# zhangyu2ustc/GCN_fmri_decoding

Hardware: AMD Instinct MI355X
Metric: fMRI-windows/sec (fwd+bwd) 6-layer ChebNet K=5 N≈10k; HBM GB/s vs roofline (higher is better)
Workload: dtype f32; 1 GPU; BASELINE configs[1]: ChebNet K=5 x6 conv (F=32, p=1, b2relu), FC 512-256-22, synthetic N=10000 kNN-8 graph -> M=10466, block_dura=15, batch 64 per GPU; global_batch=64, parallelism=dp1, step=fwd+loss+bwd+allreduce+Adam, batch gathered on device

## Files before the change

### gcn_fmri_decoding_amd/_lib.py

```python
import ctypes as C
import os

_HERE = os.path.dirname(os.path.abspath(__file__))
LIB_PATH = os.environ.get('CHEBGCN_LIB') or os.path.join(_HERE, 'libchebgcn.so')

BIAS_NONE, BIAS_FILTER, BIAS_VERTEX = 0, 1, 2
POOL_MAX, POOL_AVG = 0, 1
KNN_EUCLIDEAN, KNN_COSINE, KNN_CORRELATION, KNN_DOT = 0, 1, 2, 3
KNN_KMAX = 32
PARCEL_MEAN, PARCEL_SUM = 0, 1


class ChebgcnError(RuntimeError):
    pass


_p = C.c_void_p
_i = C.c_int
_i64 = C.c_int64
_f = C.c_float

SIGNATURES = {
    'chebgcn_version': (_i, []),
    'chebgcn_last_error': (C.c_char_p, []),
    'chebgcn_last_dispatch': (C.c_char_p, []),
    'chebgcn_plane_stride': (_i, [_i]),
    'chebgcn_graph_create': (_i, [_i, _i64, _p, _p, _p, C.POINTER(_p)]),
    'chebgcn_graph_create_planes': (_i, [_i, _i64, _p, _p, _p, _i, C.POINTER(_p)]),
    'chebgcn_graph_destroy': (None, [_p]),
    'chebgcn_graph_query': (_i, [_p, _i, C.POINTER(_i64)]),
    'chebgcn_recurrence_fwd': (_i, [_p, _p, _p, _i, _i, _i, _p]),
    'chebgcn_recurrence_bwd': (_i, [_p, _p, _p, _i, _i, _i, _p]),
    'chebgcn_recurrence_fwd_t': (_i, [_p, _p, _p, _i, _i, _i, _p]),
    'chebgcn_reindex_weights': (_i, [_p, _p, _i, _i, _i, _p]),
    'chebgcn_reindex_weights_batch': (_i, [_i, _p, _p, _p, _p, _p, _p]),
    'chebgcn_contract_fwd': (_i, [_p, _p, _p, _i, _p, _p, _i, _i, _i, _i, _i, _i, _i, _i, _p]),
    'chebgcn_contract_fwd_windows_supported': (_i, [_i, _i, _i, _i, _i, _i]),
    'chebgcn_contract_fwd_windows': (_i, [_p, _i64, _p, _p, _p, _i, _p, _p, _i, _i, _i, _i, _i, _i, _i, _i, _p]),
    'chebgcn_contract_fwd_bf16_workspace': (C.c_size_t, [_i, _i, _i]),
    'chebgcn_contract_fwd_bf16': (_i, [_p, _p, _p, _i, _p, _p, _i, _i, _i, _i, _i, _i, _i, _i, _i, _p, C.c_size_t, _p]),
    'chebgcn_contract_bwd_x_bf16_workspace': (C.c_size_t, [_i, _i, _i]),
    'chebgcn_contract_bwd_x_bf16': (_i, [_p, _p, _p, _i, _i, _i, _i, _i, _i, _p, C.c_size_t, _p]),
    'chebgcn_contract_bwd_w_bf16_workspace': (C.c_size_t, [_i, _i, _i, _i, _i]),
    'chebgcn_contract_bwd_w_bf16': (_i, [_p, _p, _p, _p, C.c_size_t, _i, _i, _i, _i, _i, _i, _p]),
    'chebgcn_adam_partials': (_i, [_i64]),
    'chebgcn_adam_step_sq': (_i, [_p, _p, _p, _p, _i64, _f, _p, _f, _f, _f, _f, _f, _p, _p]),
    'chebgcn_adam_step_sq_all': (_i, [_p, _p, _p, _p, _i64, _i64, _f, _p, _f, _f, _f, _f, _f, _p, _p]),
    'chebgcn_nadam_step_sq_all': (_i, [_p, _p, _p, _p, _i64, _i64, _f, _p, _f, _f, _f, _f, _f, _p, _p]),
    'chebgcn_loss_bookkeeping': (_i, [_p, _p, _i, _f, _p, _f, _f, _p, _p, _p, _p]),
    'chebgcn_set_scalars': (_i, [_p, C.c_float, C.c_float, _p]),
    'chebgcn_softmax_xent': (_i, [_p, _p, _i, _p, _p, _i, _i, _p]),
    'chebgcn_relu_grad_bf16': (_i, [_p, _p, _p, _p, _i, _i, _i, _i, _p, C.c_size_t, _p]),
    'chebgcn_bf16_dy16_supported': (_i, [_i, _i, _i, _i, _i]),
    'chebgcn_contract_bwd_w_bf16_dy16': (_i, [_p, _p, _p, _p, C.c_size_t, _i, _i, _i, _i, _i, _p]),
    'chebgcn_contract_bwd_x_bf16_dy16': (_i, [_p, _p, _p, _i, _i, _i, _i, _i, _p, C.c_size_t, _p]),
    'chebgcn_brelu_pool_fwd': (_i, [_p, _p, _i, _p, _p, _i, _i, _i, _i, _i, _i, _p]),
    'chebgcn_brelu_pool_bwd_workspace': (C.c_size_t, [_i, _i, _i, _i, _i]),
    'chebgcn_brelu_pool_bwd': (_i, [_p, _p, _p, _p, _p, _i, _i, _i, _i, _i, _i, _i, _p, C.c_size_t, _p]),
    'chebgcn_pool_gather_fwd': (_i, [_p, _p, _p, _p, _i, _i, _i, _i, _i, _i, _p]),
    'chebgcn_pool_scatter_bwd_workspace': (C.c_size_t, [_i, _i, _i, _i, _i]),
    'chebgcn_pool_scatter_bwd': (_i, [_p, _p, _p, _p, _p, _i, _i, _i, _i, _i, _i, _i, _p, C.c_size_t, _p]),
    'chebgcn_contract_bwd_w_workspace': (C.c_size_t, [_i, _i, _i, _i, _i]),
    'chebgcn_contract_bwd_w': (_i, [_p, _p, _p, _p, C.c_size_t, _i, _i, _i, _i, _i, _p]),
    'chebgcn_contract_bwd_x': (_i, [_p, _p, _p, _i, _i, _i, _i, _i, _p]),
    'chebgcn_contract_bwd_x_relu': (_i, [_p, _p, _p, _p, _i, _i, _i, _i, _i, _p]),
    'chebgcn_contract_bwd_w_relu': (_i, [_p, _p, _p, _p, _p, C.c_size_t, _i, _i, _i, _i, _i, _p]),
    'chebgcn_contract_bwd_w_relu_bias_merged': (_i, [_i, _i, _i, _i, _i]),
    'chebgcn_contract_bwd_w_relu_bias': (_i, [_p, _p, _p, _p, _p, _p, C.c_size_t, _i, _i, _i, _i, _i, _p]),
    'chebgcn_contract_fwd_mean_supported': (_i, [_i, _i, _i, _i, _i]),
    'chebgcn_contract_fwd_gated_supported': (_i, [_i, _i, _i, _i, _i]),
    'chebgcn_contract_fwd_gated': (_i, [_p, _p, _p, _p, _i, _i, _i, _i, _i, _p]),
    'chebgcn_contract_fwd_mean': (_i, [_p, _p, _p, _i, _p, _p, _i, _i, _i, _i, _i, _p]),
    'chebgcn_contract_bwd_w_relu_mean': (_i, [_p, _p, _p, _p, _p, C.c_size_t, _i, _i, _i, _i, _i, _p]),
    'chebgcn_contract_bwd_x_relu_mean': (_i, [_p, _p, _p, _p, _i, _i, _i, _i, _i, _p]),
    'chebgcn_bias_grad_relu_mean': (_i, [_p, _p, _p, _i, _i, _i, _i, _p, C.c_size_t, _p]),
    'chebgcn_relu_grad_mean': (_i, [_p, _p, _p, _p, _i, _i, _i, _i, _p, C.c_size_t, _p]),
    'chebgcn_fused_layer_supported': (_i, [_p, _i, _i, _i, _i]),
    'chebgcn_fused_layer_workspace': (C.c_size_t, [_p, _i, _i, _i, _i]),
    'chebgcn_fused_layer_fwd': (_i, [_p, _p, _p, _p, _i, _p, _p, _p, _p, C.c_size_t, _i, _i, _i, _i, _i, _p]),
    'chebgcn_fused_layer_bwd_x': (_i, [_p, _p, _p, _p, _p, _i, _i, _i, _i, _p]),
    'chebgcn_perm_data': (_i, [_p, _p, _p, _p, _i, _i, _i, _i, _p]),
    'chebgcn_to_plane': (_i, [_p, _p, _i, _i, _i, _p]),
    'chebgcn_from_plane': (_i, [_p, _p, _i, _i, _i, _p]),
    'chebgcn_feature_mean_fwd': (_i, [_p, _p, _i, _i, _i, _p]),
    'chebgcn_feature_mean_bwd': (_i, [_p, _p, _i, _i, _i, _p]),
    'chebgcn_fc_fwd_supported': (_i, [_i, _i, _i]),
    'chebgcn_fc_fwd_workspace': (C.c_size_t, [_i, _i, _i]),
    'chebgcn_fc_fwd': (_i, [_p, _i64, _p, _p, _p, _p, C.c_size_t, _i, _i, _i, _i, _p]),
    'chebgcn_fc_bwd': (_i, [_p, _i64, _p, _p, _p, _p, _p, _p, _i64, _i, _i, _i, _p]),
    'chebgcn_planes_to_rows': (_i, [_p, _p, _p, _i, _i, _i, _i64, _p]),
    'chebgcn_rows_to_planes': (_i, [_p, _p, _p, _i, _i, _i, _i64, _p]),
    'chebgcn_adam_step': (_i, [_p, _p, _p, _p, _i64, _f, _f, _f, _f, _f, _f, _p]),
    'chebgcn_adam_step_dev': (_i, [_p, _p, _p, _p, _i64, _p, _f, _f, _f, _f, _f, _p]),
    'chebgcn_metis_one_level_f32': (_i, [_i64, _p, _p, _p, _p, _p, _i64, _p]),
    'chebgcn_metis_one_level_f32p': (_i, [_i64, _p, _p, _p, _p, _p, _i64, _p]),
    'chebgcn_metis_one_level_f64': (_i, [_i64, _p, _p, _p, _p, _p, _i64, _p]),
    'chebgcn_compute_perm_level': (_i, [_p, _i64, _p, _i64, _p]),
    'chebgcn_bank_order': (_i, [_i, _p, _p, _i, _p, _p]),
    'chebgcn_spectral_transform': (_i, [_p, _p, _p, _i, _i, _i, _p]),
    'chebgcn_spectral_mix_fwd': (_i, [_p, _p, _p, _i, _i, _i, _i, _p]),
    'chebgcn_spectral_mix_bwd_x': (_i, [_p, _p, _p, _i, _i, _i, _i, _p]),
    'chebgcn_spectral_mix_bwd_w': (_i, [_p, _p, _p, _i, _i, _i, _i, _p]),
    'chebgcn_spectral_spline_expand': (_i, [_p, _p, _p, _i, _i, _i, _p]),
    'chebgcn_spectral_spline_expand_bwd': (_i, [_p, _p, _p, _i, _i, _i, _p]),
    'chebgcn_saliency_supported': (_i, [_i]),
    'chebgcn_saliency_seed': (_i, [_p, _p, _i, _i, _i, _p, _p, _i, _i, _p]),
    'chebgcn_saliency_path': (_i, [_p, _p, _p, _p, _p, _i, _i, _i, _i, _i, _i, _p]),
    'chebgcn_saliency_reduce': (_i, [_p, _p, _p, _p, _p, _i, _i, _i, _i, _i, _i, _p, _p, _i, _p, _p]),
    'chebgcn_occlusion_supported': (_i, [_i]),
    'chebgcn_occlusion_rows': (_i, [_p, _p, _p, _p, _p, _i64, _i, _i, _i, _i, _i, _i, _p]),
    'chebgcn_occlusion_score': (_i, [_p, _i64, _i, _i, _i, _i, _p, _i, _p, _p, _p]),
    'chebgcn_occlusion_class_sums': (_i, [_p, _p, _i, _i, _i, _p, _p]),
    'chebgcn_gradcam_weights': (_i, [_p, _i, _i, _i, _p, _p]),
    'chebgcn_gradcam_map': (_i, [_p, _p, _p, _p, _i, _i, _i, _i, _i, _p, _i64, _p]),
    'chebgcn_gather_windows': (_i, [_p, _i64, _p, _p, _p, _p, _p, _i, _i, _i, _p]),
    'chebgcn_gather_windows_mix': (_i, [_p, _i64, _p, _p, _i, _p, _p, _p, _p, _i, _i, _i, _p]),
    'chebgcn_window_stats_workspace': (C.c_size_t, [_i64, _i, _i]),
    'chebgcn_window_stats': (_i, [_p, _i64, _p, _i64, _p, _p, _p, _p, _i, _i, _p, C.c_size_t, _p]),
    'chebgcn_gather_windows_indexed': (_i, [_p, _i64, _p, _i64, _i, _i, _p, _p, _i64, _i, _p, _p, _p, _p, _i, _i, _i, _p]),
    'chebgcn_window_stats_indexed_workspace': (C.c_size_t, [_i64, _i, _i]),
    'chebgcn_window_stats_indexed': (_i, [_p, _i64, _p, _i64, _i, _i, _p, _p, _p, _p, _i, _i, _p, C.c_size_t, _p]),
    'chebgcn_knn_workspace': (C.c_size_t, [_i, _i, _i]),
    'chebgcn_knn': (_i, [_p, _i, _i, _i, _i, _p, _p, _p, C.c_size_t, _p]),
    'chebgcn_series_normalise': (_i, [_p, _i64, _p, _i, _i, _f, _p, _p]),
    'chebgcn_parcellate_query': (_i, [_i]),
    'chebgcn_parcellate': (_i, [_p, _i64, _p, _p, _i64, _p, _p, _i64, _i64, _i, _i, _i, _p]),
    'chebgcn_parcel_expand': (_i, [_p, _p, _p, _i64, _i, _i, _f, _p]),
}

_lib = None


def lib():
    global _lib
    if _lib is None:
        if not os.path.exists(LIB_PATH):
            raise ChebgcnError(
                'libchebgcn.so not found at %s: build it with '
                '`python -c "import __graft_entry__ as g; g.build()"` or '
                '`make -C gcn_fmri_decoding_amd/csrc` (needs hipcc, --offload-arch=gfx950). '
                'There is no CPU fallback.' % LIB_PATH)
        import torch
        handle = C.CDLL(LIB_PATH)
        for name, (res, args) in SIGNATURES.items():
            fn = getattr(handle, name)
            fn.restype = res
            fn.argtypes = args
        _lib = handle
    return _lib


dispatch_log = None


def check(rc, what):
    if rc != 0:
        msg = lib().chebgcn_last_error()
        raise ChebgcnError('%s failed (%d): %s' % (what, rc, msg.decode() if msg else '?'))
    if dispatch_log is not None:
        dispatch_log.append((what, lib().chebgcn_last_dispatch().decode()))


def last_dispatch():
    return lib().chebgcn_last_dispatch().decode()


def plane_stride(M):
    return (int(M) + 31) & ~31
```

### gcn_fmri_decoding_amd/csrc/head.hip

```cpp
#include <hip/hip_runtime.h>
#include "../../include/chebgcn.h"
#include "status.h"
#include "contract_common.h"

namespace chebgcn {

constexpr int FC_WAVES = 8;
constexpr int FC_CHUNK = 32;
constexpr int FC_U = 2;

__global__ void __launch_bounds__(FC_WAVES * 64)
fc_fwd_kernel(const float* __restrict__ x, long long ldx, const float* __restrict__ W, const float* __restrict__ bias,
              float* __restrict__ y, float* __restrict__ part_out, int B, int I, int O, int relu, int cps) {
    __shared__ float part[FC_WAVES][32][33];
    const int lane = threadIdx.x & 63, wave = threadIdx.x >> 6;
    const int c = lane & 31, h = lane >> 5;
    const int bx = blockIdx.x, by = blockIdx.y, bz = blockIdx.z;
    const int o0 = bx * 32, b0 = by * 32;
    const int brow = min(b0 + c, B - 1), ocol = min(o0 + c, O - 1);
    const float* xr = x + (size_t)brow * ldx;
    const float* wc = W + ocol;
    const int nchunks = (I + FC_CHUNK - 1) / FC_CHUNK;
    const int q_lo = bz * cps, q_hi = min(q_lo + cps, nchunks);
    f32x16 acc;
// ... 97 lines not shown
                const int b = 8 * (wave + FC_WAVES * (q0 + u)) + 4 * h + j;
                const bool ok = b < B;
                const float gm = (ok && yv[u][j] > 0.f) ? gv[u][j] : 0.f;
                bsum += gm;
                acc = __builtin_amdgcn_mfma_f32_32x32x2f32(ok ? av[u][j] : 0.f, gm, acc, 0, 0, 0);
            }
    }
#pragma unroll
    for (int j = 0; j < 16; ++j) part[wave][acc_row(j, h)][c] = acc[j];
    bpart[wave][h][c] = bsum;
    __syncthreads();
    for (int e = threadIdx.x; e < 32 * 32; e += FC_WAVES * 64) {
        const int r = e >> 5, cc = e & 31;
        float s = part[0][r][cc];
#pragma unroll
        for (int w = 1; w < FC_WAVES; ++w) s += part[w][r][cc];
        if (i0 + r < I && o0 + cc < O) dW[(size_t)(i0 + r) * O + o0 + cc] = s;
    }
    if (db && blockIdx.y == 0 && threadIdx.x < 32 && o0 + threadIdx.x < O) {
        float s = 0.f;
#pragma unroll
        for (int w = 0; w < FC_WAVES; ++w) s += bpart[w][0][threadIdx.x] + bpart[w][1][threadIdx.x];
        db[o0 + threadIdx.x] = s;
    }
}

template <bool VEC>
__global__ void __launch_bounds__(FC_WAVES * 64)
fc_bwd_x_kernel(const float* __restrict__ g, const float* __restrict__ y, const float* __restrict__ W,
                float* __restrict__ dx, long long lddx, int B, int I, int O) {
    __shared__ float part[FC_WAVES][32][33];
    const int lane = threadIdx.x & 63, wave = threadIdx.x >> 6;
    const int c = lane & 31, h = lane >> 5;
    const int i0 = blockIdx.x * 32, b0 = blockIdx.y * 32;
    const int brow = min(b0 + c, B - 1), irow = min(i0 + c, I - 1);
    const float* gr = g + (size_t)brow * O;
    const float* yr = y ? y + (size_t)brow * O : nullptr;
    const float* wr = W + (size_t)irow * O;
    const int nchunks = (O + 7) >> 3;
    f32x16 acc;
#pragma unroll
    for (int j = 0; j < 16; ++j) acc[j] = 0.f;
    constexpr int U = 4;
    for (int q0 = 0; wave + FC_WAVES * q0 < nchunks; q0 += U) {
        f32x4 gv[U], yv[U], wv[U];
#pragma unroll
        for (int u = 0; u < U; ++u) {
            const int k = 8 * (wave + FC_WAVES * (q0 + u)) + 4 * h;
            if (VEC) {
                const int kc = k < O ? k : 0;
                gv[u] = *reinterpret_cast<const f32x4*>(gr + kc);
                wv[u] = *reinterpret_cast<const f32x4*>(wr + kc);
                if (yr) yv[u] = *reinterpret_cast<const f32x4*>(yr + kc);
            } else {
#pragma unroll
                for (int j = 0; j < 4; ++j) {
                    const int kc = k + j < O ? k + j : 0;
                    gv[u][j] = gr[kc];
                    wv[u][j] = wr[kc];
                    if (yr) yv[u][j] = yr[kc];
                }
            }
        }
#pragma unroll
        for (int u = 0; u < U; ++u) {
            const int k = 8 * (wave + FC_WAVES * (q0 + u)) + 4 * h;
#pragma unroll
            for (int j = 0; j < 4; ++j) {
                const bool ok = k + j < O;
                const float gm = (ok && (!yr || yv[u][j] > 0.f)) ? gv[u][j] : 0.f;
                acc = __builtin_amdgcn_mfma_f32_32x32x2f32(gm, ok ? wv[u][j] : 0.f, acc, 0, 0, 0);
            }
        }
    }
#pragma unroll
    for (int j = 0; j < 16; ++j) part[wave][acc_row(j, h)][c] = acc[j];
    __syncthreads();
    for (int e = threadIdx.x; e < 32 * 32; e += FC_WAVES * 64) {
        const int r = e >> 5, cc = e & 31;
        float s = part[0][r][cc];
#pragma unroll
        for (int w = 1; w < FC_WAVES; ++w) s += part[w][r][cc];
        if (b0 + r < B && i0 + cc < I) dx[(size_t)(b0 + r) * lddx + i0 + cc] = s;
    }
}

constexpr int FLAT_V = 64;
template <bool TO_ROWS>
__global__ void __launch_bounds__(256)
planes_rows_kernel(const float* __restrict__ src, float* __restrict__ dst, const int* __restrict__ order, int M, int Mp, int F,
                   long long ldr) {
    __shared__ float tile[32][FLAT_V + 1];
    const int b = blockIdx.y, v0 = blockIdx.x * FLAT_V;
    const int nv = max(0, min(FLAT_V, M - v0));
    const int nall = min(FLAT_V, Mp - v0);
    for (int f0 = 0; f0 < F; f0 += 32) {
        const int nf = min(32, F - f0);
        if (TO_ROWS) {
            for (int e = threadIdx.x; e < 32 * FLAT_V; e += 256) {
                const int f = e / FLAT_V, vl = e % FLAT_V;
                if (f < nf && vl < nv) tile[f][vl] = src[((size_t)b * F + f0 + f) * Mp + v0 + vl];
            }
            __syncthreads();
            for (int e = threadIdx.x; e < nf * nv; e += 256) {
                const int vl = e / nf, f = e % nf;
                const int m = order ? order[v0 + vl] : v0 + vl;
                dst[(size_t)b * ldr + (size_t)m * F + f0 + f] = tile[f][vl];
            }
        } else {
            for (int e = threadIdx.x; e < nf * nv; e += 256) {
                const int vl = e / nf, f = e % nf;
                const int m = order ? order[v0 + vl] : v0 + vl;
                tile[f][vl] = src[(size_t)b * ldr + (size_t)m * F + f0 + f];
            }
            __syncthreads();
            for (int e = threadIdx.x; e < 32 * FLAT_V; e += 256) {
                const int f = e / FLAT_V, vl = e % FLAT_V;
                if (f < nf && vl < nall) dst[((size_t)b * F + f0 + f) * Mp + v0 + vl] = vl < nv ? tile[f][vl] : 0.f;
            }
        }
        __syncthreads();
    }
}

}

namespace chebgcn {
constexpr int XENT_REG = 32;
template <typename LabelT>
__global__ void __launch_bounds__(256)
softmax_xent_kernel(const float* __restrict__ z, const LabelT* __restrict__ y, float* __restrict__ loss,
                    float* __restrict__ dz, int B, int C) {
    __shared__ float part[256];
    float acc = 0.f;
    const float invB = 1.f / (float)B;
    for (int b = threadIdx.x; b < B; b += 256) {
        const float* row = z + (size_t)b * C;
        long long t = (long long)y[b];
        const bool bad = t < 0 || t >= C;
        t = t < 0 ? 0 : t >= C ? C - 1 : t;
        float* drow = dz + (size_t)b * C;
        if (bad) {
            acc += __builtin_nanf("");
            for (int c = 0; c < C; ++c) drow[c] = __builtin_nanf("");
            continue;
        }
        if (C <= XENT_REG) {
            float v[XENT_REG];
#pragma unroll
            for (int c = 0; c < XENT_REG; ++c) v[c] = c < C ? row[c] : -__builtin_inff();
            float m = v[0];
#pragma unroll
            for (int c = 1; c < XENT_REG; ++c) m = fmaxf(m, v[c]);
            float s = 0.f, so = 0.f, et = 0.f;
#pragma unroll
            for (int c = 0; c < XENT_REG; ++c) {
                v[c] = c < C ? expf(v[c] - m) : 0.f;
                s += v[c];
                so += c == t ? 0.f : v[c];
                et = c == t ? v[c] : et;
            }
            acc += et > 1e-30f ? log1pf(so / et) : logf(s) - logf(fmaxf(et, 1e-45f));
            const float inv = invB / s;
#pragma unroll
            for (int c = 0; c < XENT_REG; ++c)
                if (c < C) drow[c] = c == t ? -so * inv : v[c] * inv;
// ... 6 lines not shown
            const float e = expf(row[c] - m);
            s += e;
            so += c == t ? 0.f : e;
        }
        const float et = expf(row[t] - m);
        acc += et > 1e-30f ? log1pf(so / et) : logf(s) - (row[t] - m);
        const float inv = invB / s;
        for (int c = 0; c < C; ++c) drow[c] = c == t ? -so * inv : expf(row[c] - m) * inv;
    }
    part[threadIdx.x] = acc;
    __syncthreads();
    for (int d = 128; d > 0; d >>= 1) {
        if ((int)threadIdx.x < d) part[threadIdx.x] += part[threadIdx.x + d];
        __syncthreads();
    }
    if (threadIdx.x == 0) *loss = part[0] * invB;
}
}

using namespace chebgcn;

static int fc_splits(int B, int I, int O) {
    const int tiles = ((O + 31) / 32) * ((B + 31) / 32);
    int s = 512 / tiles;
    const int by_len = (I + 511) / 512;
    if (s > by_len) s = by_len;
    return s < 1 ? 1 : s;
}

extern "C" int chebgcn_fc_fwd_supported(int B, int I, int O) {
    return B > 0 && I > 0 && O > 0 && I <= (1 << 20) && (long long)B * O <= (1 << 20);
}

extern "C" size_t chebgcn_fc_fwd_workspace(int B, int I, int O) {
    if (!chebgcn_fc_fwd_supported(B, I, O)) return 0;
    const int S = fc_splits(B, I, O);
    return S > 1 ? (size_t)S * B * O * sizeof(float) : 0;
}

extern "C" int chebgcn_fc_fwd(const float* x, int64_t ldx, const float* W, const float* bias, float* y, void* workspace,
                              size_t workspace_bytes, int B, int I, int O, int relu, chebgcn_stream stream_) {
    hipStream_t stream = (hipStream_t)stream_;
    CG_REQUIRE(x && W && y && B > 0 && I > 0 && O > 0 && ldx >= I, "fc_fwd: bad argument");
    if (!chebgcn_fc_fwd_supported(B, I, O) || (ldx & 3) || ((uintptr_t)x & 15))
        return CHEBGCN_EUNSUPPORTED;
    const int S = fc_splits(B, I, O);
    const int nchunks = (I + FC_CHUNK - 1) / FC_CHUNK, cps = (nchunks + S - 1) / S;
    CG_REQUIRE(S == 1 || (workspace && workspace_bytes >= chebgcn_fc_fwd_workspace(B, I, O)), "fc_fwd: workspace too small");
    dim3 grid((O + 31) / 32, (B + 31) / 32, S);
    note_dispatch(S > 1 ? "fc_fwd_kernel<split>" : "fc_fwd_kernel");
    if (S > 1) note_dispatch_more("fc_fwd_reduce_kernel");
    hipLaunchKernelGGL(fc_fwd_kernel, grid, dim3(FC_WAVES * 64), 0, stream, x, (long long)ldx, W, bias, y,
                       S > 1 ? (float*)workspace : nullptr, B, I, O, relu, cps);
    if (S > 1)
        hipLaunchKernelGGL(fc_fwd_reduce_kernel, dim3((B * O + 255) / 256), dim3(256), 0, stream, (const float*)workspace, bias,
                           y, B * O, O, S, relu);
    CG_HIP(hipGetLastError());
    return CHEBGCN_OK;
}

extern "C" int chebgcn_fc_bwd(const float* x, int64_t ldx, const float* W, const float* g, const float* y, float* dW,
                              float* db, float* dx, int64_t lddx, int B, int I, int O, chebgcn_stream stream_) {
    hipStream_t stream = (hipStream_t)stream_;
    CG_REQUIRE(x && W && g && B > 0 && I > 0 && O > 0 && ldx >= I && (!dx || lddx >= I), "fc_bwd: bad argument");
    if (!chebgcn_fc_fwd_supported(B, I, O)) return CHEBGCN_EUNSUPPORTED;
    note_dispatch(dW ? "fc_bwd_w_kernel" : "");
    if (dW) {
        dim3 grid((O + 31) / 32, (I + 31) / 32);
        hipLaunchKernelGGL(fc_bwd_w_kernel, grid, dim3(FC_WAVES * 64), 0, stream, x, (long long)ldx, g, y, dW, db, B, I, O);
    }
    if (dx) {
        dim3 grid((I + 31) / 32, (B + 31) / 32);
        const bool vec = (O & 3) == 0 && ((uintptr_t)g & 15) == 0 && ((uintptr_t)W & 15) == 0 && (!y || ((uintptr_t)y & 15) == 0);
        note_dispatch_more(vec ? "fc_bwd_x_kernel<true>" : "fc_bwd_x_kernel<false>");
        if (vec)
            hipLaunchKernelGGL(fc_bwd_x_kernel<true>, grid, dim3(FC_WAVES * 64), 0, stream, g, y, W, dx, (long long)lddx, B, I, O);
        else
            hipLaunchKernelGGL(fc_bwd_x_kernel<false>, grid, dim3(FC_WAVES * 64), 0, stream, g, y, W, dx, (long long)lddx, B, I, O);
    }
    CG_HIP(hipGetLastError());
    return CHEBGCN_OK;
}

static int planes_rows(bool to_rows, const float* src, float* dst, const int32_t* order, int B, int M, int F, int64_t ldr,
                       hipStream_t stream) {
    CG_REQUIRE(src && dst && B > 0 && B <= 65535 && M > 0 && F > 0 && ldr >= (int64_t)M * F,
               to_rows ? "planes_to_rows: bad argument" : "rows_to_planes: bad argument");
    const int Mp = plane_stride(M);
    dim3 grid(((to_rows ? M : Mp) + FLAT_V - 1) / FLAT_V, B);
    note_dispatch(to_rows ? "planes_rows_kernel<to_rows>" : "planes_rows_kernel<to_planes>");
    if (to_rows)
        hipLaunchKernelGGL(planes_rows_kernel<true>, grid, dim3(256), 0, stream, src, dst, order, M, Mp, F, (long long)ldr);
    else
        hipLaunchKernelGGL(planes_rows_kernel<false>, grid, dim3(256), 0, stream, src, dst, order, M, Mp, F, (long long)ldr);
    CG_HIP(hipGetLastError());
    return CHEBGCN_OK;
}

extern "C" int chebgcn_planes_to_rows(const float* planes, float* rows, const int32_t* order, int B, int M, int F, int64_t ldr,
                                      chebgcn_stream stream) {
    return planes_rows(true, planes, rows, order, B, M, F, ldr, (hipStream_t)stream);
}

extern "C" int chebgcn_rows_to_planes(const float* rows, float* planes, const int32_t* order, int B, int M, int F, int64_t ldr,
                                      chebgcn_stream stream) {
    return planes_rows(false, rows, planes, order, B, M, F, ldr, (hipStream_t)stream);
}

extern "C" int chebgcn_softmax_xent(const float* logits, const void* labels, int labels_int64, float* loss, float* dlogits,
                                    int B, int C, chebgcn_stream stream_) {
    hipStream_t stream = (hipStream_t)stream_;
    CG_REQUIRE(logits && labels && loss && dlogits, "softmax_xent: NULL argument");
    CG_REQUIRE(B > 0 && C > 0, "softmax_xent: bad shape");
    note_dispatch(labels_int64 ? "softmax_xent_kernel<int64>" : "softmax_xent_kernel<int32>");
    if (labels_int64)
        hipLaunchKernelGGL(softmax_xent_kernel<long long>, dim3(1), dim3(256), 0, stream, logits, (const long long*)labels, loss,
                           dlogits, B, C);
    else
        hipLaunchKernelGGL(softmax_xent_kernel<int32_t>, dim3(1), dim3(256), 0, stream, logits, (const int32_t*)labels, loss,
                           dlogits, B, C);
    CG_HIP(hipGetLastError());
    return CHEBGCN_OK;
}
```

### gcn_fmri_decoding_amd/ops.py

```python
import ctypes as C
import os
import weakref

import numpy as np
import scipy.sparse as sp
import torch

from . import _lib
from . import graph as _graph
from ._lib import BIAS_FILTER, BIAS_NONE, BIAS_VERTEX, POOL_AVG, POOL_MAX, plane_stride


def _stream():
    return C.c_void_p(torch.cuda.current_stream().cuda_stream)


def _p(t):
    return C.c_void_p(t.data_ptr()) if t is not None else None


class KernelTimers:

    def __init__(self, every=1, by_dispatch=False):
        self.records = {}
# ... 1001 lines not shown
    return out


def spectral_mix_bwd_w(dyh, xh, M):
    B, Fout, Mp = dyh.shape
    Fin = xh.shape[1]
    dW = torch.empty((M, Fout, Fin), dtype=torch.float32, device=dyh.device)
    _launch('spectral_mix_bwd_w', 4.0 * (B * (Fin + Fout) * Mp + dW.numel()), 2.0 * B * M * Fin * Fout,
            lambda: _lib.check(_lib.lib().chebgcn_spectral_mix_bwd_w(_p(dyh), _p(xh), _p(dW), B, M, Fin, Fout, _stream()),
                               'spectral_mix_bwd_w'))
    return dW


def spline_expand(Bs, Wk, transpose=False):
    M, K = Bs.shape
    C = Wk.shape[1]
    if transpose:
        out = torch.empty((K, C), dtype=torch.float32, device=Wk.device)
        fn, what = _lib.lib().chebgcn_spectral_spline_expand_bwd, 'spectral_spline_expand_bwd'
    else:
        out = torch.empty((M, C), dtype=torch.float32, device=Wk.device)
        fn, what = _lib.lib().chebgcn_spectral_spline_expand, 'spectral_spline_expand'
    _launch(what, 4.0 * (M * K + (M + K) * C), 2.0 * M * K * C,
            lambda: _lib.check(fn(_p(Bs), _p(Wk), _p(out), M, K, C, _stream()), what))
    return out


class SpectralConv(torch.autograd.Function):

    @staticmethod
    def forward(ctx, x, W, basis, Bs, M, Fout):
        _require_cuda(x, W, basis, Bs)
        x = x if x.is_contiguous() else x.contiguous()
        B, Fin, Mp = x.shape
        if basis.shape != (Mp, Mp):
            raise ValueError('spectral conv: basis %s for planes of %d vertices' % (tuple(basis.shape), M))
        Wd = W.detach().contiguous()
        Wf = (spline_expand(Bs, Wd) if Bs is not None else Wd).view(M, Fout, Fin)
        xh = spectral_transform(x, basis, M, False)
        y = spectral_transform(spectral_mix(xh, Wf, M), basis, M, True)
        ctx.save_for_backward(xh if ctx.needs_input_grad[1] else None, Wf, basis, Bs)
        ctx.M = M
        return y

    @staticmethod
    def backward(ctx, gy):
        xh, Wf, basis, Bs = ctx.saved_tensors
        M = ctx.M
        gy = gy if gy.is_contiguous() else gy.contiguous()
        dyh = spectral_transform(gy, basis, M, False)
        dx = dW = None
        if ctx.needs_input_grad[1]:
            dW = spectral_mix_bwd_w(dyh, xh, M)
            if Bs is not None:
                dW = spline_expand(Bs, dW.view(M, -1), transpose=True)
        if ctx.needs_input_grad[0]:
            dx = spectral_transform(spectral_mix(dyh, Wf, M, transpose=True), basis, M, True)
        return dx, dW, None, None, None, None


class FeatureMean(torch.autograd.Function):

    @staticmethod
    def forward(ctx, x, M):
        _require_cuda(x)
        x = x if x.is_contiguous() else x.contiguous()
        B, F, Mp = x.shape
        y = torch.empty((B, M), dtype=torch.float32, device=x.device)
        _lib.check(_lib.lib().chebgcn_feature_mean_fwd(_p(x), _p(y), B, M, F, _stream()), 'feature_mean_fwd')
        ctx.cfg = (B, M, F, Mp)
        return y

    @staticmethod
    def backward(ctx, gy):
        B, M, F, Mp = ctx.cfg
        gy = gy.contiguous()
        dx = torch.empty((B, F, Mp), dtype=torch.float32, device=gy.device)
        _lib.check(_lib.lib().chebgcn_feature_mean_bwd(_p(gy), _p(dx), B, M, F, _stream()), 'feature_mean_bwd')
        return dx, None


FC_BWD_MAX_INNER = int(os.environ.get('CHEBGCN_FC_BWD_MAX_INNER', 4096))
FC_FWD_MAX_INNER = int(os.environ.get('CHEBGCN_FC_FWD_MAX_INNER', 1 << 20))


def fc_forward(x, W, b, relu):
    if not (x.is_cuda and x.dtype == torch.float32 and W.dtype == torch.float32 and x.dim() == 2 and W.is_contiguous()
            and x.stride(1) == 1 and x.stride(0) % 4 == 0 and x.data_ptr() % 16 == 0):
        return None
    B, I = x.shape
    O = W.shape[1]
    L = _lib.lib()
    if I > FC_FWD_MAX_INNER or not L.chebgcn_fc_fwd_supported(B, I, O):
        return None
    y = torch.empty((B, O), dtype=torch.float32, device=x.device)
    nws = L.chebgcn_fc_fwd_workspace(B, I, O)
    ws = _workspace(nws, x.device, 'fc_fwd') if nws else None
    _lib.check(L.chebgcn_fc_fwd(_p(x), x.stride(0), _p(W), _p(b), _p(y), _p(ws), nws, B, I, O, 1 if relu else 0, _stream()),
               'fc_fwd')
    return y


def fc_backward(x, W, g, y, dW, db, need_dx):
    B, I = x.shape
    O = W.shape[1]
    L = _lib.lib()
    if not (x.is_cuda and x.dtype == torch.float32 and x.stride(1) == 1 and W.is_contiguous() and g.is_contiguous()
            and dW.is_contiguous() and db.is_contiguous() and (y is None or y.is_contiguous())
            and I <= FC_BWD_MAX_INNER and L.chebgcn_fc_fwd_supported(B, I, O)):
        return None
    dx = torch.empty((B, I), dtype=torch.float32, device=x.device) if need_dx else None
    _lib.check(L.chebgcn_fc_bwd(_p(x), x.stride(0), _p(W), _p(g), _p(y), _p(dW), _p(db), _p(dx), I, B, I, O, _stream()),
               'fc_bwd')
    return (dx,)


def adam_step_sq_all(p, g, m, v, n_reg, lr_t, sq_partials, beta1=0.9, beta2=0.999, eps=1e-8, grad_scale=1.0, l2=0.0):
    _require_cuda(p, g, m, v, sq_partials)
    n = p.numel()
    if not (g.numel() == m.numel() == v.numel() == n) or n == 0 or not (0 <= n_reg <= n):
        raise ValueError('adam_step_sq_all: size mismatch')
    lib = _lib.lib()
    nparts = lib.chebgcn_adam_partials(n)
    if sq_partials.dtype != torch.float32 or sq_partials.numel() < nparts:
        raise ValueError('adam_step_sq_all: sq_partials needs %d float32' % nparts)
    dev_lr = isinstance(lr_t, torch.Tensor)
    if dev_lr and (lr_t.dtype != torch.float32 or lr_t.numel() != 1 or not lr_t.is_cuda):
        raise ValueError('adam_step_sq_all: a device lr_t must be one float32')
    _lib.check(lib.chebgcn_adam_step_sq_all(_p(p), _p(g), _p(m), _p(v), n, int(n_reg), 0.0 if dev_lr else float(lr_t),
                                            _p(lr_t) if dev_lr else None, float(beta1), float(beta2), float(eps), float(grad_scale),
                                            float(l2), _p(sq_partials), _stream()), 'adam_step_sq_all')
    return nparts


def nadam_step_sq_all(p, g, m, v, n_reg, lr_t, sq_partials, beta1=0.9, beta2=0.999, eps=1e-8, grad_scale=1.0, l2=0.0):
    _require_cuda(p, g, m, v, sq_partials)
    n = p.numel()
    if not (g.numel() == m.numel() == v.numel() == n) or n == 0 or not (0 <= n_reg <= n):
        raise ValueError('nadam_step_sq_all: size mismatch')
    lib = _lib.lib()
    nparts = lib.chebgcn_adam_partials(n)
    if sq_partials.dtype != torch.float32 or sq_partials.numel() < nparts:
        raise ValueError('nadam_step_sq_all: sq_partials needs %d float32' % nparts)
    dev_lr = isinstance(lr_t, torch.Tensor)
    if dev_lr and (lr_t.dtype != torch.float32 or lr_t.numel() != 1 or not lr_t.is_cuda):
        raise ValueError('nadam_step_sq_all: a device lr_t must be one float32')
    n_bytes = 28.0 * n
    _lib.check(_launch('nadam', n_bytes, 0.0, lambda: lib.chebgcn_nadam_step_sq_all(
        _p(p), _p(g), _p(m), _p(v), n, int(n_reg), 0.0 if dev_lr else float(lr_t), _p(lr_t) if dev_lr else None, float(beta1),
        float(beta2), float(eps), float(grad_scale), float(l2), _p(sq_partials), _stream())), 'nadam_step_sq_all')
    return nparts


def planes_to_rows(planes, M, order=None, ld=None):
    _require_cuda(planes)
    B, F, Mp = planes.shape
    if Mp != plane_stride(M) or not planes.is_contiguous():
        raise ValueError('planes_to_rows: planes of %d vertices expected' % M)
    ld = ld or ((M * F + 3) & ~3)
    rows = torch.empty((B, ld), dtype=torch.float32, device=planes.device)
    _lib.check(_launch('planes_to_rows', 8.0 * B * M * F, 0.0, lambda: _lib.lib().chebgcn_planes_to_rows(
        _p(planes), _p(rows), _p(order), B, M, F, ld, _stream())), 'planes_to_rows')
    return rows


def rows_to_planes(rows, M, F, order=None):
    _require_cuda(rows)
    B, ld = rows.shape
    if ld < M * F or rows.stride(1) != 1 or rows.stride(0) != ld:
        raise ValueError('rows_to_planes: rows of at least %d floats expected' % (M * F))
    planes = torch.empty((B, F, plane_stride(M)), dtype=torch.float32, device=rows.device)
    _lib.check(_launch('rows_to_planes', 8.0 * B * M * F, 0.0, lambda: _lib.lib().chebgcn_rows_to_planes(
        _p(rows), _p(planes), _p(order), B, M, F, ld, _stream())), 'rows_to_planes')
    return planes


class FlatFC(torch.autograd.Function):

    @staticmethod
    def forward(ctx, x, W, b, order, M, relu, gW, gb):
        _require_cuda(x, W, b)
        B, F, Mp = x.shape
        I, O = M * F, W.shape[1]
        if tuple(W.shape) != (I, O) or tuple(b.shape) != (O,):
            raise ValueError('FlatFC: weights [%d, O] and bias [O] expected' % I)
        L = _lib.lib()
        if not L.chebgcn_fc_fwd_supported(B, I, O):
            raise ValueError('FlatFC: %d x %d x %d is outside the range of chebgcn_fc_fwd' % (B, I, O))
        rows = planes_to_rows(x.contiguous(), M, order)
        ld = rows.shape[1]
        Wc, bc = W.detach().contiguous(), b.detach().contiguous()
        y = torch.empty((B, O), dtype=torch.float32, device=x.device)
        nws = L.chebgcn_fc_fwd_workspace(B, I, O)
# ... 230 lines not shown
```

### include/chebgcn.h

```cpp
#ifndef CHEBGCN_H
#define CHEBGCN_H

#include <stddef.h>
#include <stdint.h>

#ifdef __cplusplus
extern "C" {
#endif

#define CHEBGCN_VERSION 1

enum {
    CHEBGCN_OK = 0,
    CHEBGCN_EINVAL = -1,
    CHEBGCN_EHIP = -2,
    CHEBGCN_ENOMEM = -3,
    CHEBGCN_EUNSUPPORTED = -4
};

enum { CHEBGCN_BIAS_NONE = 0, CHEBGCN_BIAS_FILTER = 1 , CHEBGCN_BIAS_VERTEX = 2  };
enum { CHEBGCN_POOL_MAX = 0, CHEBGCN_POOL_AVG = 1 };

typedef struct chebgcn_graph chebgcn_graph;
typedef void* chebgcn_stream;
// ... 53 lines not shown

int chebgcn_relu_grad_bf16(const float* dout, const uint8_t* relu_mask, uint16_t* dy16, float* dbias, int bias_kind,
                           int B, int M, int F, void* workspace, size_t workspace_bytes, chebgcn_stream stream);
int chebgcn_bf16_dy16_supported(int B, int M, int Fin, int K, int Fout);
int chebgcn_contract_bwd_w_bf16_dy16(const float* stack, const uint16_t* dy16, float* dW, void* workspace,
                                     size_t workspace_bytes, int B, int M, int Fin, int K, int Fout,
                                     chebgcn_stream stream);
int chebgcn_contract_bwd_x_bf16_dy16(const uint16_t* dy16, const float* W, float* gstack, int B, int M, int Fin,
                                     int K, int Fout, void* workspace, size_t workspace_bytes, chebgcn_stream stream);

int chebgcn_brelu_pool_fwd(const float* x, const float* bias, int bias_kind, float* out,
                           uint8_t* argmax, int B, int M, int F, int pool, int pool_kind,
                           int relu, chebgcn_stream stream);

size_t chebgcn_brelu_pool_bwd_workspace(int B, int M, int F, int pool, int bias_kind);
int chebgcn_brelu_pool_bwd(const float* dout, const float* out, const uint8_t* argmax,
                           float* dy, float* dbias, int bias_kind, int B, int M, int F,
                           int pool, int pool_kind, int relu, void* workspace, size_t workspace_bytes,
                           chebgcn_stream stream);

int chebgcn_pool_gather_fwd(const float* y, const int32_t* pmap, float* out, uint8_t* sel, int B, int M, int F,
                            int pool, int pool_kind, int relu, chebgcn_stream stream);
size_t chebgcn_pool_scatter_bwd_workspace(int B, int M, int F, int pool, int bias_kind);
int chebgcn_pool_scatter_bwd(const float* dout, const uint8_t* sel, const int32_t* smap, float* dy, float* dbias,
                             int bias_kind, int B, int M, int F, int pool, int pool_kind, int relu, void* workspace,
                             size_t workspace_bytes, chebgcn_stream stream);

size_t chebgcn_contract_bwd_w_workspace(int B, int M, int Fin, int K, int Fout);
int chebgcn_contract_bwd_w(const float* stack, const float* dy, float* dW, void* workspace,
                           size_t workspace_bytes, int B, int M, int Fin, int K, int Fout,
                           chebgcn_stream stream);
int chebgcn_contract_bwd_w_relu(const float* stack, const float* dout, const uint8_t* relu_mask,
                                float* dW, void* workspace, size_t workspace_bytes, int B, int M,
                                int Fin, int K, int Fout, chebgcn_stream stream);
int chebgcn_contract_bwd_w_relu_bias_merged(int B, int M, int Fin, int K, int Fout);
int chebgcn_contract_bwd_w_relu_bias(const float* stack, const float* dout, const uint8_t* relu_mask,
                                     float* dW, float* dbias, void* workspace, size_t workspace_bytes,
                                     int B, int M, int Fin, int K, int Fout, chebgcn_stream stream);
int chebgcn_contract_bwd_x_relu(const float* dout, const uint8_t* relu_mask, const float* W,
                                float* gstack, int B, int M, int Fin, int K, int Fout,
                                chebgcn_stream stream);
int chebgcn_contract_bwd_x(const float* dy, const float* W, float* gstack, int B, int M,
                           int Fin, int K, int Fout, chebgcn_stream stream);

int chebgcn_contract_fwd_mean_supported(int B, int M, int Fin, int K, int Fout);
int chebgcn_contract_fwd_mean(const float* stack, const float* W, const float* bias, int bias_kind,
                              float* mean_out, uint8_t* relu_mask, int B, int M, int Fin, int K, int Fout,
                              chebgcn_stream stream);
int chebgcn_contract_bwd_w_relu_mean(const float* stack, const float* gmean, const uint8_t* relu_mask,
                                     float* dW, void* workspace, size_t workspace_bytes, int B, int M,
                                     int Fin, int K, int Fout, chebgcn_stream stream);
int chebgcn_contract_bwd_x_relu_mean(const float* gmean, const uint8_t* relu_mask, const float* W,
                                     float* gstack, int B, int M, int Fin, int K, int Fout,
                                     chebgcn_stream stream);
int chebgcn_bias_grad_relu_mean(const float* gmean, const uint8_t* relu_mask, float* dbias, int bias_kind,
                                int B, int M, int F, void* workspace, size_t workspace_bytes,
                                chebgcn_stream stream);
int chebgcn_relu_grad_mean(const float* gmean, const uint8_t* relu_mask, float* dy, float* dbias, int bias_kind,
                           int B, int M, int F, void* workspace, size_t workspace_bytes,
                           chebgcn_stream stream);

int chebgcn_fused_layer_supported(const chebgcn_graph* g, int B, int Fin, int K, int Fout);
size_t chebgcn_fused_layer_workspace(const chebgcn_graph* g, int B, int Fin, int K, int Fout);
int chebgcn_fused_layer_fwd(const chebgcn_graph* g, const float* x, const float* W, const float* bias, int bias_kind,
                            float* stack, float* out, uint8_t* relu_mask, void* workspace, size_t workspace_bytes,
                            int B, int Fin, int K, int Fout, int relu, chebgcn_stream stream);
int chebgcn_fused_layer_bwd_x(const chebgcn_graph* g, const float* dout, const uint8_t* relu_mask, const float* W,
                              float* dx, int B, int Fin, int K, int Fout, chebgcn_stream stream);

int chebgcn_perm_data(const float* x, const int32_t* perm, const int32_t* sample, float* out,
                      int S, int N, int M, int F, chebgcn_stream stream);
int chebgcn_to_plane(const float* x_bmf, float* out_plane, int B, int M, int F, chebgcn_stream stream);
int chebgcn_from_plane(const float* x_plane, float* out_bmf, int B, int M, int F, chebgcn_stream stream);

int chebgcn_feature_mean_fwd(const float* x, float* y, int B, int M, int F, chebgcn_stream stream);
int chebgcn_feature_mean_bwd(const float* dy, float* dx, int B, int M, int F, chebgcn_stream stream);

int chebgcn_fc_fwd_supported(int B, int I, int O);
size_t chebgcn_fc_fwd_workspace(int B, int I, int O);
int chebgcn_fc_fwd(const float* x, int64_t ldx, const float* W, const float* bias, float* y, void* workspace,
                   size_t workspace_bytes, int B, int I, int O, int relu, chebgcn_stream stream);
int chebgcn_fc_bwd(const float* x, int64_t ldx, const float* W, const float* g, const float* y, float* dW, float* db,
                   float* dx, int64_t lddx, int B, int I, int O, chebgcn_stream stream);

int chebgcn_planes_to_rows(const float* planes, float* rows, const int32_t* order, int B, int M, int F, int64_t ldr,
                           chebgcn_stream stream);
int chebgcn_rows_to_planes(const float* rows, float* planes, const int32_t* order, int B, int M, int F, int64_t ldr,
                           chebgcn_stream stream);

int chebgcn_set_scalars(float* dst, float v0, float v1, chebgcn_stream stream);

int chebgcn_adam_partials(int64_t n);
int chebgcn_adam_step_sq(float* p, const float* g, float* m, float* v, int64_t n, float lr_t, const float* lr_t_dev,
                         float beta1, float beta2, float eps, float grad_scale, float l2, float* sq_partials,
                         chebgcn_stream stream);
int chebgcn_adam_step_sq_all(float* p, const float* g, float* m, float* v, int64_t n, int64_t n_reg, float lr_t,
                             const float* lr_t_dev, float beta1, float beta2, float eps, float grad_scale, float l2,
                             float* sq_partials, chebgcn_stream stream);
int chebgcn_nadam_step_sq_all(float* p, const float* g, float* m, float* v, int64_t n, int64_t n_reg, float lr_t,
                              const float* lr_t_dev, float beta1, float beta2, float eps, float grad_scale, float l2,
                              float* sq_partials, chebgcn_stream stream);
int chebgcn_loss_bookkeeping(const float* cross_entropy, const float* sq_partials, int nparts, float half_reg, float* ema,
                             float decay, float corr, const float* corr_dev, float* loss_out, float* loss_average_out,
                             chebgcn_stream stream);

int chebgcn_softmax_xent(const float* logits, const void* labels, int labels_int64, float* loss, float* dlogits, int B,
                         int C, chebgcn_stream stream);

int chebgcn_adam_step(float* p, const float* g, float* m, float* v, int64_t n, float lr_t,
                      float beta1, float beta2, float eps, float grad_scale, float l2,
                      chebgcn_stream stream);
int chebgcn_adam_step_dev(float* p, const float* g, float* m, float* v, int64_t n, const float* lr_t_dev,
                          float beta1, float beta2, float eps, float grad_scale, float l2,
                          chebgcn_stream stream);

int chebgcn_metis_one_level_f32(int64_t nnz, const int64_t* rr, const int64_t* cc, const float* vv,
                                const int64_t* rid, const float* weights, int64_t N, int32_t* cluster_id);
int chebgcn_metis_one_level_f32p(int64_t nnz, const int64_t* rr, const int64_t* cc, const float* vv,
                                 const int64_t* rid, const float* weights, int64_t N, int32_t* cluster_id);
int chebgcn_metis_one_level_f64(int64_t nnz, const int64_t* rr, const int64_t* cc, const double* vv,
                                const int64_t* rid, const double* weights, int64_t N, int32_t* cluster_id);
int chebgcn_compute_perm_level(const int32_t* parent, int64_t n_fine, const int64_t* order,
                               int64_t n_order, int64_t* out);


int chebgcn_spectral_transform(const float* in, const float* basis, float* out, int R, int M, int transpose,
                               chebgcn_stream stream);
int chebgcn_spectral_mix_fwd(const float* xh, const float* W, float* yh, int B, int M, int Fin, int Fout,
                             chebgcn_stream stream);
int chebgcn_spectral_mix_bwd_x(const float* dyh, const float* W, float* dxh, int B, int M, int Fin, int Fout,
                               chebgcn_stream stream);
int chebgcn_spectral_mix_bwd_w(const float* dyh, const float* xh, float* dW, int B, int M, int Fin, int Fout,
                               chebgcn_stream stream);
int chebgcn_spectral_spline_expand(const float* Bs, const float* Wk, float* W, int M, int K, int C, chebgcn_stream stream);
int chebgcn_spectral_spline_expand_bwd(const float* Bs, const float* dW, float* dWk, int M, int K, int C,
                                       chebgcn_stream stream);

enum { CHEBGCN_SCORE_LOGIT = 0, CHEBGCN_SCORE_LOGPROB = 1 };
int chebgcn_saliency_supported(int F);
enum { CHEBGCN_SAL_GRADIENT = 0, CHEBGCN_SAL_GRAD_X_INPUT = 1, CHEBGCN_SAL_INTEGRATED = 2 };
int chebgcn_saliency_seed(const float* logits, const int64_t* targets, int rep, int nvalid, int score, float* dlogits,
                          int64_t* cls_out, int B, int C, chebgcn_stream stream);
int chebgcn_saliency_path(const float* x, const int32_t* perm, const int32_t* sample, const float* baseline, float* out, int nw,
                          int steps, int R, int N, int M, int F, chebgcn_stream stream);
int chebgcn_saliency_reduce(const float* dx, const float* x, const int32_t* perm, const int32_t* sample, const float* baseline,
                            int nw, int steps, int M, int F, int method, int absolute, float* out, const int64_t* cls, int ncls,
                            double* acc, chebgcn_stream stream);

int chebgcn_occlusion_supported(int F);
int chebgcn_occlusion_rows(const float* x, const int32_t* perm, const int32_t* gid, const float* baseline, float* out, int64_t r0,
                           int R, int S, int G, int N, int M, int F, chebgcn_stream stream);
int chebgcn_occlusion_score(const float* logits, int64_t r0, int R, int S, int G, int C, const int64_t* cls, int score, float* ref,
                            float* drop, chebgcn_stream stream);
int chebgcn_occlusion_class_sums(const float* drop, const int64_t* cls, int S, int G, int ncls, double* acc,
                                 chebgcn_stream stream);

int chebgcn_gradcam_weights(const float* G, int nw, int F, int N, float* alpha, chebgcn_stream stream);
int chebgcn_gradcam_map(const float* A, const float* G, const float* alpha, const int32_t* order, int nw, int F, int N, int P,
                        int relu, float* out, int64_t ldo, chebgcn_stream stream);

int chebgcn_gather_windows(const float* series, int64_t Ttot, const int64_t* rows, const int32_t* sample, const float* scale,
                           const float* shift, float* out, int B, int M, int C, chebgcn_stream stream);
int chebgcn_gather_windows_mix(const float* series, int64_t Ttot, const int64_t* rows, const int32_t* cnt, int smax,
                               const int32_t* sample, const float* scale, const float* shift, float* out, int B, int M, int C,
                               chebgcn_stream stream);
size_t chebgcn_window_stats_workspace(int64_t Ttot, int M, int C);
// ... 41 lines not shown
```

Baseline: 21600 windows/s.

## Add persistent fused FC backward kernel for large inner dimension

Adds a new FC backward kernel for the first FC layer, where the inner dimension is huge (flattened graph features, about 10k×32) and the output is 512. The kernel stages the ReLU-masked output gradient for the whole batch in LDS once per block. Each block then loops persistently over 32-row tiles of I, computing dW and dx with MFMA, and block 0 also produces db. Before this, such layers fell back to the generic PyTorch path because of the FC_BWD_MAX_INNER limit. The kernel uses a large dynamic LDS allocation and caps the grid at the CU count, so latency hiding depends on a single block per CU.

```diff
diff --git a/gcn_fmri_decoding_amd/_lib.py b/gcn_fmri_decoding_amd/_lib.py
--- a/gcn_fmri_decoding_amd/_lib.py
+++ b/gcn_fmri_decoding_amd/_lib.py
@@ -88,6 +88,8 @@
     'chebgcn_fc_fwd_workspace': (C.c_size_t, [_i, _i, _i]),
     'chebgcn_fc_fwd': (_i, [_p, _i64, _p, _p, _p, _p, C.c_size_t, _i, _i, _i, _i, _p]),
     'chebgcn_fc_bwd': (_i, [_p, _i64, _p, _p, _p, _p, _p, _p, _i64, _i, _i, _i, _p]),
+    'chebgcn_fc_bwd_large_supported': (_i, [_i, _i, _i]),
+    'chebgcn_fc_bwd_large': (_i, [_p, _i64, _p, _p, _p, _p, _p, _p, _i64, _i, _i, _i, _p]),
     'chebgcn_planes_to_rows': (_i, [_p, _p, _p, _i, _i, _i, _i64, _p]),
     'chebgcn_rows_to_planes': (_i, [_p, _p, _p, _i, _i, _i, _i64, _p]),
     'chebgcn_adam_step': (_i, [_p, _p, _p, _p, _i64, _f, _f, _f, _f, _f, _f, _p]),
diff --git a/gcn_fmri_decoding_amd/csrc/head.hip b/gcn_fmri_decoding_amd/csrc/head.hip
--- a/gcn_fmri_decoding_amd/csrc/head.hip
+++ b/gcn_fmri_decoding_amd/csrc/head.hip
@@ -203,6 +203,125 @@
 #pragma unroll
         for (int w = 1; w < FC_WAVES; ++w) s += part[w][r][cc];
         if (b0 + r < B && i0 + cc < I) dx[(size_t)(b0 + r) * lddx + i0 + cc] = s;
+    }
+}
+
+constexpr int FCL_TI = 32;
+constexpr int FCL_GS = 512 + 4;
+constexpr int FCL_B = 64, FCL_O = 512;
+constexpr size_t FCL_LDS = (size_t)FCL_B * FCL_GS * sizeof(float);
+
+__global__ void __launch_bounds__(FC_WAVES * 64)
+fc_bwd_large_kernel(const float* __restrict__ x, long long ldx, const float* __restrict__ W, const float* __restrict__ g,
+                    const float* __restrict__ y, float* __restrict__ dW, float* __restrict__ db, float* __restrict__ dx,
+                    long long lddx, int B, int I, int O, int nitems) {
+    extern __shared__ float fcl_lds[];
+    float* gs = fcl_lds;
+    float (*part)[32][33] = reinterpret_cast<float (*)[32][33]>(fcl_lds);
+    float (*xs)[33] = reinterpret_cast<float (*)[33]>(fcl_lds + FC_WAVES * 32 * 33);
+    const int lane = threadIdx.x & 63, wave = threadIdx.x >> 6;
+    const int c = lane & 31, h = lane >> 5;
+    const int ow = wave * 64;
+    for (int e = threadIdx.x; e < FCL_B * (FCL_O / 4); e += FC_WAVES * 64) {
+        const int b = e / (FCL_O / 4), o = 4 * (e % (FCL_O / 4));
+        f32x4 v = {0.f, 0.f, 0.f, 0.f};
+        if (b < B && o < O) {
+            v = *reinterpret_cast<const f32x4*>(g + (size_t)b * O + o);
+            if (y) {
+                const f32x4 yv = *reinterpret_cast<const f32x4*>(y + (size_t)b * O + o);
+#pragma unroll
+                for (int j = 0; j < 4; ++j) v[j] = yv[j] > 0.f ? v[j] : 0.f;
+            }
+        }
+        *reinterpret_cast<f32x4*>(gs + b * FCL_GS + o) = v;
+    }
+    __syncthreads();
+    float gw[2][32];
+    f32x4 gt[2][8];
+#pragma unroll
+    for (int t = 0; t < 2; ++t)
+#pragma unroll
+        for (int q = 0; q < 32; ++q) gw[t][q] = gs[(2 * q + h) * FCL_GS + ow + 32 * t + c];
+#pragma unroll
+    for (int bt = 0; bt < 2; ++bt)
+#pragma unroll
+        for (int Q = 0; Q < 8; ++Q) gt[bt][Q] = *reinterpret_cast<const f32x4*>(gs + (32 * bt + c) * FCL_GS + ow + 8 * Q + 4 * h);
+    if (db && blockIdx.x == 0 && (int)threadIdx.x < O) {
+        float s = 0.f;
+        for (int b = 0; b < B; ++b) s += gs[b * FCL_GS + threadIdx.x];
+        db[threadIdx.x] = s;
+    }
+    __syncthreads();
+    const int nbt = B > 32 ? 2 : 1;
+    for (int item = blockIdx.x; item < nitems; item += gridDim.x) {
+        const int i0 = item * FCL_TI;
+        const bool irow_ok = i0 + c < I;
+        f32x4 wv[8];
+        if (dx) {
+            const float* wr = W + (size_t)(irow_ok ? i0 + c : 0) * O;
+#pragma unroll
+            for (int Q = 0; Q < 8; ++Q) {
+                const int o = ow + 8 * Q + 4 * h;
+                const f32x4 t = *reinterpret_cast<const f32x4*>(wr + (o < O ? o : 0));
+                const bool ok = irow_ok && o < O;
+#pragma unroll
+                for (int j = 0; j < 4; ++j) wv[Q][j] = ok ? t[j] : 0.f;
+            }
+        }
+        for (int e = threadIdx.x; e < FCL_B * FCL_TI; e += FC_WAVES * 64) {
+            const int b = e >> 5, ii = e & 31;
+            xs[b][ii] = (b < B && i0 + ii < I) ? x[(size_t)b * ldx + i0 + ii] : 0.f;
+        }
+        __syncthreads();
+        if (dW && ow < O) {
+            f32x16 acc[2];
+#pragma unroll
+            for (int t = 0; t < 2; ++t)
+#pragma unroll
+                for (int j = 0; j < 16; ++j) acc[t][j] = 0.f;
+#pragma unroll
+            for (int q = 0; q < 32; ++q) {
+                const float a = xs[2 * q + h][c];
+#pragma unroll
+                for (int t = 0; t < 2; ++t) acc[t] = __builtin_amdgcn_mfma_f32_32x32x2f32(a, gw[t][q], acc[t], 0, 0, 0);
+            }
+#pragma unroll
+            for (int t = 0; t < 2; ++t) {
+                const int o = ow + 32 * t + c;
+#pragma unroll
+                for (int j = 0; j < 16; ++j) {
+                    const int r = i0 + acc_row(j, h);
+                    if (r < I && o < O) dW[(size_t)r * O + o] = acc[t][j];
+                }
+            }
+        }
+        if (dx) {
+#pragma unroll
+            for (int bt = 0; bt < 2; ++bt) {
+                if (bt >= nbt) break;
+                f32x16 acc;
+#pragma unroll
+                for (int j = 0; j < 16; ++j) acc[j] = 0.f;
+#pragma unroll
+                for (int Q = 0; Q < 8; ++Q)
+#pragma unroll
+                    for (int j = 0; j < 4; ++j)
+                        acc = __builtin_amdgcn_mfma_f32_32x32x2f32(gt[bt][Q][j], wv[Q][j], acc, 0, 0, 0);
+#pragma unroll
+                for (int j = 0; j < 16; ++j) part[wave][acc_row(j, h)][c] = acc[j];
+                __syncthreads();
+                for (int e = threadIdx.x; e < 32 * 32; e += FC_WAVES * 64) {
+                    const int r = e >> 5, cc = e & 31;
+                    float s = part[0][r][cc];
+#pragma unroll
+                    for (int w = 1; w < FC_WAVES; ++w) s += part[w][r][cc];
+                    if (32 * bt + r < B && i0 + cc < I) dx[(size_t)(32 * bt + r) * lddx + i0 + cc] = s;
+                }
+                __syncthreads();
+            }
+        } else {
+            __syncthreads();
+        }
     }
 }
 
@@ -375,6 +494,42 @@
     return CHEBGCN_OK;
 }
 
+static int fcl_num_cus() {
+    static int cus = 0;
+    if (cus == 0) {
+        int dev = 0, n = 0;
+        cus = (hipGetDevice(&dev) == hipSuccess &&
+               hipDeviceGetAttribute(&n, hipDeviceAttributeMultiprocessorCount, dev) == hipSuccess && n > 0) ? n : 256;
+    }
+    return cus;
+}
+
+extern "C" int chebgcn_fc_bwd_large_supported(int B, int I, int O) {
+    return B > 0 && B <= FCL_B && O > 0 && O <= FCL_O && (O & 3) == 0 && I > 0 && I <= (1 << 20);
+}
+
+extern "C" int chebgcn_fc_bwd_large(const float* x, int64_t ldx, const float* W, const float* g, const float* y, float* dW,
+                                    float* db, float* dx, int64_t lddx, int B, int I, int O, chebgcn_stream stream_) {
+    hipStream_t stream = (hipStream_t)stream_;
+    CG_REQUIRE(x && W && g && B > 0 && I > 0 && O > 0 && ldx >= I && (!dx || lddx >= I), "fc_bwd_large: bad argument");
+    CG_REQUIRE(dW || dx, "fc_bwd_large: nothing to compute");
+    if (!chebgcn_fc_bwd_large_supported(B, I, O) || ((uintptr_t)g & 15) || ((uintptr_t)W & 15) || (y && ((uintptr_t)y & 15)))
+        return CHEBGCN_EUNSUPPORTED;
+    const int nitems = (I + FCL_TI - 1) / FCL_TI;
+    const int grid = nitems < fcl_num_cus() ? nitems : fcl_num_cus();
+    static bool lds_set = false;
+    if (!lds_set) {
+        CG_HIP(hipFuncSetAttribute(reinterpret_cast<const void*>(fc_bwd_large_kernel), hipFuncAttributeMaxDynamicSharedMemorySize,
+                                   (int)FCL_LDS));
+        lds_set = true;
+    }
+    note_dispatch("fc_bwd_large_kernel");
+    hipLaunchKernelGGL(fc_bwd_large_kernel, dim3(grid), dim3(FC_WAVES * 64), FCL_LDS, stream, x, (long long)ldx, W, g, y, dW,
+                       dW ? db : nullptr, dx, (long long)lddx, B, I, O, nitems);
+    CG_HIP(hipGetLastError());
+    return CHEBGCN_OK;
+}
+
 static int planes_rows(bool to_rows, const float* src, float* dst, const int32_t* order, int B, int M, int F, int64_t ldr,
                        hipStream_t stream) {
     CG_REQUIRE(src && dst && B > 0 && B <= 65535 && M > 0 && F > 0 && ldr >= (int64_t)M * F,
diff --git a/gcn_fmri_decoding_amd/ops.py b/gcn_fmri_decoding_amd/ops.py
--- a/gcn_fmri_decoding_amd/ops.py
+++ b/gcn_fmri_decoding_amd/ops.py
@@ -1107,6 +1107,7 @@
 
 FC_BWD_MAX_INNER = int(os.environ.get('CHEBGCN_FC_BWD_MAX_INNER', 4096))
 FC_FWD_MAX_INNER = int(os.environ.get('CHEBGCN_FC_FWD_MAX_INNER', 1 << 20))
+FC_LARGE_ARMS = True
 
 
 def fc_forward(x, W, b, relu):
@@ -1132,8 +1133,16 @@
     L = _lib.lib()
     if not (x.is_cuda and x.dtype == torch.float32 and x.stride(1) == 1 and W.is_contiguous() and g.is_contiguous()
             and dW.is_contiguous() and db.is_contiguous() and (y is None or y.is_contiguous())
-            and I <= FC_BWD_MAX_INNER and L.chebgcn_fc_fwd_supported(B, I, O)):
+            and L.chebgcn_fc_fwd_supported(B, I, O)):
         return None
+    if I > FC_BWD_MAX_INNER:
+        if not (FC_LARGE_ARMS and g.dtype == torch.float32 and W.dtype == torch.float32 and L.chebgcn_fc_bwd_large_supported(B, I, O)
+                and W.data_ptr() % 16 == 0 and g.data_ptr() % 16 == 0 and (y is None or y.data_ptr() % 16 == 0)):
+            return None
+        dx = torch.empty((B, I), dtype=torch.float32, device=x.device) if need_dx else None
+        _lib.check(L.chebgcn_fc_bwd_large(_p(x), x.stride(0), _p(W), _p(g), _p(y), _p(dW), _p(db), _p(dx), I, B, I, O,
+                                          _stream()), 'fc_bwd')
+        return (dx,)
     dx = torch.empty((B, I), dtype=torch.float32, device=x.device) if need_dx else None
     _lib.check(L.chebgcn_fc_bwd(_p(x), x.stride(0), _p(W), _p(g), _p(y), _p(dW), _p(db), _p(dx), I, B, I, O, _stream()),
                'fc_bwd')
diff --git a/include/chebgcn.h b/include/chebgcn.h
--- a/include/chebgcn.h
+++ b/include/chebgcn.h
@@ -159,6 +159,9 @@
                    size_t workspace_bytes, int B, int I, int O, int relu, chebgcn_stream stream);
 int chebgcn_fc_bwd(const float* x, int64_t ldx, const float* W, const float* g, const float* y, float* dW, float* db,
                    float* dx, int64_t lddx, int B, int I, int O, chebgcn_stream stream);
+int chebgcn_fc_bwd_large_supported(int B, int I, int O);
+int chebgcn_fc_bwd_large(const float* x, int64_t ldx, const float* W, const float* g, const float* y, float* dW, float* db,
+                         float* dx, int64_t lddx, int B, int I, int O, chebgcn_stream stream);
 
 int chebgcn_planes_to_rows(const float* planes, float* rows, const int32_t* order, int B, int M, int F, int64_t ldr,
                            chebgcn_stream stream);
```

New measurement: 21710 windows/s (median of 6 runs). Within noise of the previous version (+0.5%).
